# yjpark1/multiagent_rl

Hardware: AMD Instinct MI355X
Metric: env-steps/sec, simple_spread N=6 x B envs, 1/2/4/8 MI355X (higher is better)
Workload: dtype f32

## Files before the change

multiagent_rl_amd/csrc/pw_kernels_spread_quad.hpp:

```cpp
#pragma once

#include "pw_kernels_spread.hpp"

namespace {

__device__ __forceinline__ void quad_pair_of(const int q, int &i, int &j)
{
    i = q < 5 ? 0 : q < 9 ? 1 : q < 12 ? 2 : q < 14 ? 3 : 4;
    j = q - (i == 0 ? 0 : i == 1 ? 5 : i == 2 ? 9 : i == 3 ? 12 : 14) + i + 1;
}

__device__ __forceinline__ void quad_act_fetch(const int32_t *row, const uint32_t lane_off, const uint32_t lds_slot, const uint32_t slot_read)
{
    unsigned keep;
    asm volatile("s_mov_b32 %0, m0\n\ts_mov_b32 m0, %3\n\ts_nop 0\n\tglobal_load_lds_dword %1, %2\n\ts_mov_b32 m0, %0"
                 : "=&s"(keep) : "v"(lane_off), "s"(row), "s"(lds_slot), "v"(slot_read) : "memory");
}

template <bool K1>
__device__ __forceinline__ void quad_pair_force(const float2 qi, const float2 qj, const uint32_t near_lo, const uint32_t near_span,
                                                const float dist_min, const float k, const float cf, float &Fx, float &Fy)
{
    const float dx = qi.x - qj.x, dy = qi.y - qj.y;
    const float d2 = dx * dx + dy * dy;
    const f32x2 a = {cf * dx, cf * dy};
    const bool near = __float_as_uint(d2) - near_lo >= near_span;
    const bool uni = (k >= 9.094947017729282e-13f) & (k <= 1099511627776.0f) & (cf >= 9.5367431640625e-07f) & (cf <= 128.0f);
    const bool c1 = (__float_as_uint(d2) - 0x12800000u) < (0x6C800000u - 0x12800000u);
    const bool c2 = fminf(fabsf(a.x), fabsf(a.y)) >= 8.673617379884035e-19f;
    const bool fast = near & c1 & c2 & uni;
    const bool any_cold = __builtin_amdgcn_ballot_w64(near & !fast) != 0;
    Fx = 0.0f; Fy = 0.0f;
    if (fast) {
        const float dist = sqrt_rn_core(d2);
        const float y0 = __builtin_amdgcn_rcpf(dist);
        __builtin_amdgcn_sched_barrier(0);
        const float yd = __builtin_fmaf(__builtin_fmaf(-dist, y0, 1.0f), y0, y0);
        const f32x2 Q = div_chain2(a, dist, yd);
        const float xarg = K1 ? div_chain1(-(dist - dist_min), k, div_refined_rcp(k))
                              : div_chain(-(dist - dist_min), k, div_refined_rcp(k));
        const float pen = softplus_branchless(xarg) * k;
        const f32x2 F = Q * f32x2{pen, pen};
        Fx = F.x;
        Fy = F.y;
    }
    if (__builtin_expect(any_cold, 0)) {
        if (near & !fast) collision_force_pair<true, K1>(qi.x, qi.y, qj.x, qj.y, dist_min, k, cf, Fx, Fy);
    }
}

#ifndef PW_QUAD_BARRIER
#define PW_QUAD_BARRIER(t) duo_barrier()
#endif
#ifndef PW_QUAD_ACT_AHEAD
#define PW_QUAD_ACT_AHEAD 4
#endif
#ifndef PW_QUAD_PAD_P
#define PW_QUAD_PAD_P()
#endif
#ifndef PW_QUAD_PAD_OB
#define PW_QUAD_PAD_OB()
#endif
constexpr int kQuadActAhead = PW_QUAD_ACT_AHEAD;
constexpr int kQuadN = 6, kQuadL = 6, kQuadEPP = 4, kQuadEPW = 8;
struct SpreadQuadLds { float4 *s_ring; float2 *s_ftab, *s_lmB, *s_utab; float *s_min, *s_rew; int32_t *s_act; uint32_t bytes; };
__host__ __device__ inline SpreadQuadLds spread_quad_lds(unsigned char *raw = nullptr)
{
    LdsCursor c{reinterpret_cast<float *>(raw)}; SpreadQuadLds o;
    o.s_ring = c.take<float4>(4 * kWave);
    o.s_ftab = c.take<float2>(2 * kQuadEPP * kQuadN * kQuadN);
    o.s_min = c.take<float>(kWave); o.s_rew = c.take<float>(kWave);
    o.s_lmB = c.take<float2>(kQuadEPW * kQuadL); o.s_act = c.take<int32_t>(2 * kQuadActAhead * kWave);
    o.s_utab = c.take<float2>(2 * 8);
    o.bytes = 4 * c.at; return o;
}
template <bool UNIT_MASS, bool COLL = false, bool K1 = false>
__global__ void __launch_bounds__(4 * kWave) pw_spread_quad_kernel(const StreamParams A, const int T)
{
    constexpr int N = kQuadN, L = kQuadL, D = 16, P2 = 15, EPP = kQuadEPP, EPW = kQuadEPW;
    extern __shared__ __attribute__((aligned(16))) unsigned char smem_raw[];
    const SpreadQuadLds Y = spread_quad_lds(smem_raw);

    const int wave = __builtin_amdgcn_readfirstlane((((int)threadIdx.x >> 6) + 2 * (((int)blockIdx.x >> 8) & 1)) & 3);
    const int lane = (int)threadIdx.x & 63;
    const int env0 = (int)blockIdx.x * EPW;
    const int envs_here = A.B - env0 < EPW ? A.B - env0 : EPW;
    const size_t BN = (size_t)A.B * N;

    const bool resets = A.auto_reset && A.max_episode_len > 0;
    int offs_all = A.ep_step[env0 + (lane < envs_here ? lane : 0)];
    auto next_reset_step = [&](int t_from) -> int {
        if (!resets) return 0x7fffffff;
        int rem = A.max_episode_len - 1 - (t_from + offs_all);
        rem = rem < 0 ? 0 : rem;
        int m = 0x7fffffff;
        for (int e = 0; e < envs_here; ++e) {
            const int r = __builtin_amdgcn_readlane(rem, e);
            m = r < m ? r : m;
        }
        return t_from + m;
    };
    int t_reset = next_reset_step(0);
    auto reset_step_update = [&](int t) {
        if (t + 1 + offs_all >= A.max_episode_len) offs_all = -(t + 1);
        t_reset = next_reset_step(t + 1);
    };
    int cur = 0;

    if (wave < 2) {
        __builtin_amdgcn_s_setprio(3);
        const int e0 = wave * EPP;
        const int nv = envs_here - e0 < 0 ? 0 : envs_here - e0 < EPP ? envs_here - e0 : EPP;
        if (nv == 0) {
            for (int t = 0; t < T; ++t) PW_QUAD_BARRIER(t);
            return;
        }
        const int la = lane < nv * N ? lane : 0;
        const int e4 = la / N, a = la - e4 * N;
        const int me = (e0 + e4) * N + a;
        const int env = env0 + e0 + e4;
        const uint32_t g = (uint32_t)env * (uint32_t)N + (uint32_t)a;
        const uint64_t env_id = A.env_id_base + (uint64_t)env;
        const int lp = lane < nv * P2 ? lane : 0;
        const int pe = lp / P2, pq = lp - pe * P2;
        int pi, pj;
        quad_pair_of(pq, pi, pj);
        const int ri = (e0 + pe) * N + pi, rj = (e0 + pe) * N + pj;
        float2 *ftab = Y.s_ftab + wave * (EPP * N * N);
        float2 *f_ij = ftab + (pe * N + pi) * N + (pj - 1), *f_ji = ftab + (pe * N + pj) * N + pi;
        const float2 *row = ftab + (e4 * N + a) * N;

        float px = A.pos_x[g], py = A.pos_y[g], vx = A.vel_x[g], vy = A.vel_y[g];
        int ep_off = A.ep_step[env];
        uint32_t ep_count = A.ep_count[env];
        Y.s_ring[me] = make_float4(px, py, vx, vy);
        float2 *utab = Y.s_utab + wave * 8;
        if (lane < 6) {
            const int ai = lane;
            float ux = 0.0f + ((ai == 1 ? 1.0f : 0.0f) - (ai == 2 ? 1.0f : 0.0f));
            float uy = 0.0f + ((ai == 3 ? 1.0f : 0.0f) - (ai == 4 ? 1.0f : 0.0f));
            ux *= A.sens; uy *= A.sens;
            if (A.fscale != 1.0f) { ux = A.fscale * ux; uy = A.fscale * uy; }
            utab[lane] = make_float2(ux + 0.0f, uy + 0.0f);
        }
        wave_lds_sync();
        const float k = A.contact_margin, cf = A.contact_force, dt = A.dt, damp = A.damp, mass = A.mass;
        const uint32_t near_lo = __float_as_uint(A.near_thr2), near_span = 0x7F800000u - near_lo;
        const unsigned char *act_row = reinterpret_cast<const unsigned char *>(A.act);
        const size_t act_stride = BN * sizeof(int32_t);
        const uint32_t act_off = g * (uint32_t)sizeof(int32_t);
        int32_t *act_ring = Y.s_act + wave * (kQuadActAhead * kWave);
        const uint32_t act_lds = __builtin_amdgcn_readfirstlane((uint32_t)reinterpret_cast<uintptr_t>(act_ring));
        auto fetch_act = [&](int t, uint32_t slot_read) {
            quad_act_fetch(reinterpret_cast<const int32_t *>(act_row), act_off, act_lds + (uint32_t)(t & (kQuadActAhead - 1)) * (kWave * 4), slot_read);
            act_row += t + 1 < T ? act_stride : (size_t)0;
        };
        asm volatile("" :: "v"(ep_off), "v"(ep_count), "v"(offs_all), "v"(px), "v"(py), "v"(vx), "v"(vy), "s"(t_reset));
        for (int t0 = 0; t0 < kQuadActAhead; ++t0) fetch_act(t0, 0u);
        float2 qi = *reinterpret_cast<const float2 *>(Y.s_ring + ri);
        float2 qj = *reinterpret_cast<const float2 *>(Y.s_ring + rj);
        PW_STAMP_DECL;
        for (int t = 0; t < T; ++t) {
            PW_STAMP_START;
            asm volatile("s_waitcnt vmcnt(%0)" :: "n"(kQuadActAhead - 1) : "memory");
            PW_STAMP(3);
            const uint32_t ai = (uint32_t)act_ring[(t & (kQuadActAhead - 1)) * kWave + lane];
            fetch_act(t + kQuadActAhead, ai);
            const float2 u0 = utab[ai < 5u ? ai : 5u];
            const bool two_slots = t == t_reset;
            float Fx, Fy;
            quad_pair_force<K1>(qi, qj, near_lo, near_span, A.dist_min, k, cf, Fx, Fy);
            *f_ij = make_float2(Fx, Fy);
            *f_ji = make_float2(-Fx, -Fy);
            PW_STAMP(0);
            float fx = u0.x, fy = u0.y;
            asm volatile("" ::: "memory");
#pragma unroll
            for (int j = 0; j < N - 1; ++j) {
                const float2 F = row[j];
                fx = F.x + fx;
                fy = F.y + fy;
            }
            vx = vx * damp; vy = vy * damp;
            vx = vx + div_mass<UNIT_MASS>(fx, mass) * dt;
            vy = vy + div_mass<UNIT_MASS>(fy, mass) * dt;
            px = px + vx * dt;
            py = py + vy * dt;
            int nxt = (cur + 1) & 3;
            Y.s_ring[nxt * kWave + me] = make_float4(px, py, vx, vy);
            if (__builtin_expect(two_slots, 0)) {
                if (t + 1 + ep_off >= A.max_episode_len) {
                    ep_count += 1;
                    ep_off = -(t + 1);
                    pw_reset_xy(A.seed, env_id, ep_count, (uint32_t)a, -1.0f, 1.0f, &px, &py);
                    vx = 0.f; vy = 0.f;
                }
                reset_step_update(t);
                nxt = (nxt + 1) & 3;
                Y.s_ring[nxt * kWave + me] = make_float4(px, py, vx, vy);
            }
            cur = nxt;
            asm volatile("" ::: "memory");
            qi = *reinterpret_cast<const float2 *>(Y.s_ring + cur * kWave + ri);
            qj = *reinterpret_cast<const float2 *>(Y.s_ring + cur * kWave + rj);
            PW_STAMP(1);
            PW_QUAD_PAD_P();
            PW_QUAD_BARRIER(t);
            PW_STAMP(2);
        }
        act_fetch_drain();
#ifdef PW_STAMPS
        if (blockIdx.x == 0 && wave == 0 && lane == 0)
            for (int i_ = 0; i_ < 4; ++i_) g_pw_stamps[i_] = st_acc[i_];
#endif
        A.pos_x[g] = px; A.pos_y[g] = py;
        A.vel_x[g] = vx; A.vel_y[g] = vy;
        A.ep_step[env] = T + ep_off;
        A.ep_count[env] = ep_count;
        return;
    }

    int e_local = lane / N;
    int a = lane - e_local * N;
    if (e_local >= envs_here) { e_local = 0; a = 0; }
    const int env = env0 + e_local;
    const int base = e_local * N, me = base + a;
    const uint32_t g = (uint32_t)env * (uint32_t)N + (uint32_t)a;
    const uint64_t env_id = A.env_id_base + (uint64_t)env;
    int ep_off = A.ep_step[env];
    uint32_t ep_count = A.ep_count[env];
    float olx = A.lm_x[(size_t)env * L + a], oly = A.lm_y[(size_t)env * L + a];

    if (wave == 2) {
        float own_p = 0.0f;
        int cnt_p = 0;
        uint32_t cmask_p = 0;
        float2 mine, q6[N];
        auto a_reads = [&](const int nxt) __attribute__((always_inline)) {
            const float4 *slot = Y.s_ring + nxt * kWave + base;
            mine = *reinterpret_cast<const float2 *>(slot + a);
#pragma unroll
            for (int j = 0; j < N; ++j) q6[j] = *reinterpret_cast<const float2 *>(slot + j);
        };
        float best, e0;
        int cnt;
        uint32_t cmask;
        auto a_dist = [&]() __attribute__((always_inline)) {
            const float px = mine.x, py = mine.y;
            float e2[N];
            cnt = 0; cmask = 0;
#pragma unroll
            for (int j = 0; j < N; ++j) {
                const float2 q = q6[j];
                const float dx = q.x - px, dy = q.y - py;
                const float d2 = dx * dx + dy * dy;
                cnt += d2 < A.coll_thr2 ? 1 : 0;
                if (COLL) cmask |= d2 < A.coll_thr2 ? 1u << j : 0u;
                const float ex = q.x - olx, ey = q.y - oly;
                e2[j] = ex * ex + ey * ey;
            }
            best = __builtin_fminf(__builtin_fminf(__builtin_fminf(e2[0], e2[1]), __builtin_fminf(e2[2], e2[3])),
                                   __builtin_fminf(e2[4], e2[5]));
            e0 = e2[0];
        };
        auto a_sqrt = [&]() __attribute__((always_inline)) -> float {
            const float b = e0 != e0 ? e0 : best;
            return sqrtf(b);
        };
        auto a_clock = [&](const int t, int nxt) __attribute__((always_inline)) {
            if (__builtin_expect(t == t_reset, 0)) {
                if (t + 1 + ep_off >= A.max_episode_len) {
                    ep_count += 1;
                    ep_off = -(t + 1);
                    pw_reset_xy(A.seed, env_id, ep_count, (uint32_t)(N + a), -1.0f, 1.0f, &olx, &oly);
                }
                reset_step_update(t);
                nxt = (nxt + 1) & 3;
            }
            cur = nxt;
        };
        float sh_own[L], sh_r[N], r;
        auto b_shfl_own = [&]() __attribute__((always_inline)) {
#pragma unroll
            for (int l = 0; l < L; ++l) sh_own[l] = __shfl(own_p, base + l, kWave);
        };
        auto b_reward = [&]() __attribute__((always_inline)) {
            r = 0.0f;
#pragma unroll
            for (int l = 0; l < L; ++l) r -= sh_own[l];
#pragma unroll
            for (int k2 = 0; k2 < N; ++k2) r -= k2 < cnt_p ? 1.0f : 0.0f;
#pragma unroll
            for (int i = 0; i < N; ++i) sh_r[i] = __shfl(r, base + i, kWave);
        };
        float *rew_t = A.rew, *rsh_t = A.rew_shared;
        uint64_t *coll_t = A.coll;
        auto b_store = [&]() __attribute__((always_inline)) {
            float acc = 0.0f;
#pragma unroll
            for (int i = 0; i < N; ++i) acc += sh_r[i];
            nt_store(rew_t + g, r);
            nt_store(rsh_t + env, acc);
            if (COLL) nt_store(coll_t + g, (uint64_t)cmask_p);
            rew_t += BN; rsh_t += A.B;
            if (COLL) coll_t += BN;
        };
        PW_STAMP_DECL;
        {
            PW_STAMP_START;
            PW_QUAD_BARRIER(0);
            PW_STAMP(0);
            const int nxt = (cur + 1) & 3;
            a_reads(nxt);
            a_dist();
            own_p = a_sqrt(); cnt_p = cnt; cmask_p = cmask;
            a_clock(0, nxt);
            PW_STAMP(1);
        }
        for (int t = 1; t < T; ++t) {
            PW_STAMP_START;
            PW_QUAD_BARRIER(t);
            PW_STAMP(0);
            const int nxt = (cur + 1) & 3;
            a_reads(nxt);
            b_shfl_own();
            a_dist();
            b_reward();
            const float own = a_sqrt();
            b_store();
            own_p = own; cnt_p = cnt; cmask_p = cmask;
            a_clock(t, nxt);
            PW_STAMP(1);
        }
        b_shfl_own();
        b_reward();
        b_store();
#ifdef PW_STAMPS
        if (blockIdx.x == 0 && lane == 0)
            for (int i_ = 0; i_ < 2; ++i_) g_pw_stamps[4 + i_] = st_acc[i_];
#endif
        return;
    }

    const int rows_here = envs_here * N;
    const int cgrp = lane & 3;
    const bool col0 = cgrp == 0;
    int row_u[3];
    uint32_t off_u[3];
#pragma unroll
    for (int u = 0; u < 3; ++u) {
        const int r = (lane >> 2) + 16 * u;
        const bool ok = r < rows_here;
        row_u[u] = ok ? r : 0;
        off_u[u] = (uint32_t)(ok ? lane + 64 * u : cgrp) * 16u;
    }
    float4 lm_u[3];
    auto load_landmarks = [&]() {
#pragma unroll
        for (int u = 0; u < 3; ++u)
            lm_u[u] = *reinterpret_cast<const float4 *>(Y.s_lmB + (row_u[u] / N) * L + (cgrp > 0 ? 2 * cgrp - 2 : 0));
    };
    Y.s_lmB[me] = make_float2(olx, oly);
    wave_lds_sync();
    load_landmarks();
    unsigned char *obs_t = reinterpret_cast<unsigned char *>(A.obs + ((size_t)env0 * N) * D);
    uint8_t *done_t = A.done, *term_t = A.terminal;
    const size_t obs_stride = BN * D * sizeof(float);
    const bool has_len = A.max_episode_len > 0;
    int t_term = has_len ? A.max_episode_len - 1 - ep_off : 0x7fffffff;
    PW_STAMP_DECL;
    for (int t = 0; t < T; ++t) {
        PW_STAMP_START;
        nt_store(done_t + g, (uint8_t)0);
        PW_QUAD_BARRIER(t);
        PW_STAMP(0);
        int nxt = (cur + 1) & 3;
        nt_store(term_t + env, (uint8_t)(t >= t_term ? 1 : 0));
        if (t == t_reset) {
            const bool rst = t >= t_term;
            if (rst) {
                if (A.final_obs) {
                    const float4 st = Y.s_ring[nxt * kWave + me];
                    stream_write_obs<L>(A.final_obs + ((size_t)t * BN + g) * D, L, Y.s_lmB + base, st.x, st.y, st.z, st.w);
                }
                ep_count += 1;
                ep_off = -(t + 1);
                t_term = A.max_episode_len - 1 - ep_off;
                pw_reset_xy(A.seed, env_id, ep_count, (uint32_t)(N + a), -1.0f, 1.0f, &olx, &oly);
            }
            reset_step_update(t);
            wave_lds_sync();
            if (rst) Y.s_lmB[me] = make_float2(olx, oly);
            wave_lds_sync();
            load_landmarks();
            nxt = (nxt + 1) & 3;
        }
        cur = nxt;
        const float4 *slot = Y.s_ring + nxt * kWave;
        float4 st[3];
#pragma unroll
        for (int u = 0; u < 3; ++u) st[u] = slot[row_u[u]];
        asm volatile("" :: "v"(st[0].x), "v"(st[0].y), "v"(st[0].z), "v"(st[0].w), "v"(st[1].x), "v"(st[1].y), "v"(st[1].z),
                           "v"(st[1].w), "v"(st[2].x), "v"(st[2].y), "v"(st[2].z), "v"(st[2].w));
#pragma unroll
        for (int u = 0; u < 3; ++u) {
            const float4 d = make_float4(lm_u[u].x - st[u].x, lm_u[u].y - st[u].y, lm_u[u].z - st[u].x, lm_u[u].w - st[u].y);
            const float4 o = make_float4(col0 ? st[u].z : d.x, col0 ? st[u].w : d.y, col0 ? st[u].x : d.z, col0 ? st[u].y : d.w);
            nt_store(reinterpret_cast<float4 *>(obs_t + off_u[u]), o);
        }
        obs_t += obs_stride; done_t += BN; term_t += A.B;
        PW_QUAD_PAD_OB();
        PW_STAMP(1);
    }
#ifdef PW_STAMPS
    if (blockIdx.x == 0 && lane == 0)
        for (int i_ = 0; i_ < 2; ++i_) g_pw_stamps[6 + i_] = st_acc[i_];
#endif
    A.lm_x[(size_t)env * L + a] = olx;
    A.lm_y[(size_t)env * L + a] = oly;
}

}
```

Measured before the change: 7.853 billion.

## Move collision tests from reward wave to observation wave via LDS handoff

The per-agent collision distance tests and the collision mask store move from the reward wave (wave 2) to the observation-writing waves. Counts are handed back through a double-buffered LDS slot that wave 2 reads one step later. The final step's counts are recomputed locally. The aim is to shorten the critical-path reward wave at the cost of extra LDS reads and writes in the obs waves, plus a reliance on the existing barrier ordering for the handoff.

```diff
diff --git a/multiagent_rl_amd/csrc/pw_kernels_spread_quad.hpp b/multiagent_rl_amd/csrc/pw_kernels_spread_quad.hpp
--- a/multiagent_rl_amd/csrc/pw_kernels_spread_quad.hpp
+++ b/multiagent_rl_amd/csrc/pw_kernels_spread_quad.hpp
@@ -49,6 +49,24 @@
     }
 }
 
+template <bool COLL>
+__device__ __forceinline__ void quad_coll_tests(const float2 mine, const float2 (&q6)[6], const float coll_thr2, int &cnt, uint32_t &cmask)
+{
+    cnt = 0; cmask = 0;
+#if defined(PW_EXPERIMENTS) && defined(PW_EXP_NO_COLL_TESTS)
+    cnt = 1;
+#else
+#pragma unroll
+    for (int j = 0; j < 6; ++j) {
+        const float2 q = q6[j];
+        const float dx = q.x - mine.x, dy = q.y - mine.y;
+        const float d2 = dx * dx + dy * dy;
+        cnt += d2 < coll_thr2 ? 1 : 0;
+        if (COLL) cmask |= d2 < coll_thr2 ? 1u << j : 0u;
+    }
+#endif
+}
+
 #ifndef PW_QUAD_BARRIER
 #define PW_QUAD_BARRIER(t) duo_barrier()
 #endif
@@ -234,28 +252,23 @@
     if (wave == 2) {
         float own_p = 0.0f;
         int cnt_p = 0;
-        uint32_t cmask_p = 0;
-        float2 mine, q6[N];
+        const int *cnt_w = reinterpret_cast<const int *>(Y.s_min) + lane;
+        const int cnt_span = (int)(Y.s_rew - Y.s_min);
+        int cnt_at = 0;
+        int pre_last = 0;
+        float2 q6[N];
         auto a_reads = [&](const int nxt) __attribute__((always_inline)) {
             const float4 *slot = Y.s_ring + nxt * kWave + base;
-            mine = *reinterpret_cast<const float2 *>(slot + a);
 #pragma unroll
             for (int j = 0; j < N; ++j) q6[j] = *reinterpret_cast<const float2 *>(slot + j);
+            pre_last = nxt;
         };
         float best, e0;
-        int cnt;
-        uint32_t cmask;
         auto a_dist = [&]() __attribute__((always_inline)) {
-            const float px = mine.x, py = mine.y;
             float e2[N];
-            cnt = 0; cmask = 0;
 #pragma unroll
             for (int j = 0; j < N; ++j) {
                 const float2 q = q6[j];
-                const float dx = q.x - px, dy = q.y - py;
-                const float d2 = dx * dx + dy * dy;
-                cnt += d2 < A.coll_thr2 ? 1 : 0;
-                if (COLL) cmask |= d2 < A.coll_thr2 ? 1u << j : 0u;
                 const float ex = q.x - olx, ey = q.y - oly;
                 e2[j] = ex * ex + ey * ey;
             }
@@ -294,16 +307,13 @@
             for (int i = 0; i < N; ++i) sh_r[i] = __shfl(r, base + i, kWave);
         };
         float *rew_t = A.rew, *rsh_t = A.rew_shared;
-        uint64_t *coll_t = A.coll;
         auto b_store = [&]() __attribute__((always_inline)) {
             float acc = 0.0f;
 #pragma unroll
             for (int i = 0; i < N; ++i) acc += sh_r[i];
             nt_store(rew_t + g, r);
             nt_store(rsh_t + env, acc);
-            if (COLL) nt_store(coll_t + g, (uint64_t)cmask_p);
             rew_t += BN; rsh_t += A.B;
-            if (COLL) coll_t += BN;
         };
         PW_STAMP_DECL;
         {
@@ -313,7 +323,7 @@
             const int nxt = (cur + 1) & 3;
             a_reads(nxt);
             a_dist();
-            own_p = a_sqrt(); cnt_p = cnt; cmask_p = cmask;
+            own_p = a_sqrt();
             a_clock(0, nxt);
             PW_STAMP(1);
         }
@@ -322,15 +332,25 @@
             PW_QUAD_BARRIER(t);
             PW_STAMP(0);
             const int nxt = (cur + 1) & 3;
+            cnt_p = cnt_w[cnt_at];
+            cnt_at = cnt_span - cnt_at;
             a_reads(nxt);
             b_shfl_own();
             a_dist();
             b_reward();
             const float own = a_sqrt();
             b_store();
-            own_p = own; cnt_p = cnt; cmask_p = cmask;
+            own_p = own;
             a_clock(t, nxt);
             PW_STAMP(1);
+        }
+        {
+            const float4 *slot = Y.s_ring + pre_last * kWave + base;
+            const float2 mine = *reinterpret_cast<const float2 *>(slot + a);
+#pragma unroll
+            for (int j = 0; j < N; ++j) q6[j] = *reinterpret_cast<const float2 *>(slot + j);
+            uint32_t cmask;
+            quad_coll_tests<false>(mine, q6, A.coll_thr2, cnt_p, cmask);
         }
         b_shfl_own();
         b_reward();
@@ -368,6 +388,10 @@
     const size_t obs_stride = BN * D * sizeof(float);
     const bool has_len = A.max_episode_len > 0;
     int t_term = has_len ? A.max_episode_len - 1 - ep_off : 0x7fffffff;
+    int *cnt_w = reinterpret_cast<int *>(Y.s_min) + lane;
+    const int cnt_span = (int)(Y.s_rew - Y.s_min);
+    int cnt_at = 0;
+    uint64_t *coll_t = A.coll;
     PW_STAMP_DECL;
     for (int t = 0; t < T; ++t) {
         PW_STAMP_START;
@@ -375,6 +399,13 @@
         PW_QUAD_BARRIER(t);
         PW_STAMP(0);
         int nxt = (cur + 1) & 3;
+        float2 cmine, cq6[N];
+        {
+            const float4 *pre = Y.s_ring + nxt * kWave + base;
+            cmine = *reinterpret_cast<const float2 *>(pre + a);
+#pragma unroll
+            for (int j = 0; j < N; ++j) cq6[j] = *reinterpret_cast<const float2 *>(pre + j);
+        }
         nt_store(term_t + env, (uint8_t)(t >= t_term ? 1 : 0));
         if (t == t_reset) {
             const bool rst = t >= t_term;
@@ -400,6 +431,17 @@
         float4 st[3];
 #pragma unroll
         for (int u = 0; u < 3; ++u) st[u] = slot[row_u[u]];
+        {
+            int cnt;
+            uint32_t cmask;
+            quad_coll_tests<COLL>(cmine, cq6, A.coll_thr2, cnt, cmask);
+            cnt_w[cnt_at] = cnt;
+            cnt_at = cnt_span - cnt_at;
+            if (COLL) {
+                nt_store(coll_t + g, (uint64_t)cmask);
+                coll_t += BN;
+            }
+        }
         asm volatile("" :: "v"(st[0].x), "v"(st[0].y), "v"(st[0].z), "v"(st[0].w), "v"(st[1].x), "v"(st[1].y), "v"(st[1].z),
                            "v"(st[1].w), "v"(st[2].x), "v"(st[2].y), "v"(st[2].z), "v"(st[2].w));
 #pragma unroll
```

New measurement: 8.011 billion (median of 6 runs). +2.0%, better.
